# bastienjossen/DDL25Spring

Measured on AMD Instinct MI355X. Metric: FedAvg rounds/sec + local samples/sec, ResNet-18 CIFAR-10-shape, 8 clients, higher is better.
Workload: dtype fp32; 1 GPU; model=resnet18-cifar10, global_batch=800, parallelism=fedavg-8clients-dp1, clients=8, local_batch=100, local_epochs=1, samples_per_client=6250, client_slots_per_gpu=8, hip_graphs=True, fp32_conv_math=auto

## Files before the change

csrc/include/conv_f32_core.h:

```cpp
#pragma once
#include "ddl_common.h"

struct ConvF32Args {
  const float* x;
  const float* w;
  const float* dy;
  float* out;
  float* stats;
  const float* bias;
  const float* residual;
  const float* mask;
  const float* in_scale;
  const float* in_shift;
  const float* bn_x;
  const float* bn_mean;
  const float* bn_rstd;
  const float* mask_scale;
  const float* mask_shift;
  float* partial;
  long long partial_cap;
  long long x_gs, w_gs, dy_gs, out_gs, bias_gs, res_gs;
  int G, N, H, W, C, K, R, S, P, Q, stride, pad;
  int relu, accumulate, split_k, res_sub, in_relu;
  int slots;
  float gscale;
  const void* wsplit;
  long long ws_gs;
  const float* dyb_x;
  const float* dyb_coef;
  float* dyb_out;
  int* tickets;
  long long tickets_cap;
};

enum { F_FWD = 0, F_DGRAD = 1, F_WGRAD = 2 };

struct FDiv {
  uint32_t m;
  int s;
};
__host__ __device__ inline FDiv mk_fdiv(uint32_t d) {
  FDiv f;
  if (d <= 1) { f.m = 0; f.s = 0; return f; }
  int l = 0;
  while ((1u << l) < d) ++l;
  f.m = (uint32_t)((((1ull << 32) * ((1ull << l) - d)) / d) + 1);
  f.s = l;
  return f;
}
__device__ __forceinline__ int fdv(int x, FDiv f) {
  if (f.s == 0) return x;
  const uint32_t t = __umulhi((uint32_t)x, f.m);
  return (int)((t + (((uint32_t)x - t) >> 1)) >> (f.s - 1));
}

struct FGeo {
  int Pd, Qd, Kr, nph, phase, split, nsplit, g, p0, q0, tq;
  int pa, pb, Hs, Ws, r0, s0, Rn, Sn;
};

template <int MODE, int BP, int BQ>
__device__ __forceinline__ FGeo fgeo(const ConvF32Args& a, int bx, int by, int g, int gy) {
  FGeo o;
  o.nph = (MODE == F_DGRAD && a.stride == 2) ? 4 : 1;
  o.phase = by % o.nph;
  o.split = by / o.nph;
  o.nsplit = gy / o.nph;
  o.g = g;
  o.pa = o.pb = o.r0 = o.s0 = 0;
  o.Hs = a.H; o.Ws = a.W; o.Rn = a.R; o.Sn = a.S;
  if (MODE == F_FWD) {
    o.Pd = a.K; o.Qd = a.N * a.P * a.Q; o.Kr = a.R * a.S * a.C;
  } else if (MODE == F_DGRAD) {
    o.Pd = a.C;
    if (o.nph == 4) {
      o.pa = o.phase >> 1; o.pb = o.phase & 1;
      o.Hs = (a.H - o.pa + 1) >> 1; o.Ws = (a.W - o.pb + 1) >> 1;
      o.r0 = (o.pa + a.pad) & 1; o.s0 = (o.pb + a.pad) & 1;
      o.Rn = (a.R - o.r0 + 1) >> 1; o.Sn = (a.S - o.s0 + 1) >> 1;
    }
    o.Qd = a.N * o.Hs * o.Ws;
    o.Kr = o.Rn * o.Sn * a.K;
  } else {
    o.Pd = a.K; o.Qd = a.R * a.S * a.C; o.Kr = a.N * a.P * a.Q;
  }
  const int ntp = (o.Pd + BP - 1) / BP;
  o.p0 = (bx % ntp) * BP;
  o.tq = bx / ntp;
  o.q0 = o.tq * BQ;
  return o;
}

template <int BP, int BQ>
struct Lay16 {
  static constexpr int NPQ = BP / 32, NQ = BQ / 32, QL = 16;
  static __device__ __forceinline__ int poff(int i, int lane) { return i * 16 + 4 * (lane >> 4); }
  static __device__ __forceinline__ int qoff(int j, int lane) { return j * 16 + (lane & 15); }
};
template <int BP, int BQ>
struct Lay32 {
  static constexpr int NPQ = BP / 16, NQ = BQ / 64, QL = 32;
  static __device__ __forceinline__ int poff(int i, int lane) {
    return (i >> 2) * 32 + 8 * (i & 3) + 4 * (lane >> 5);
  }
  static __device__ __forceinline__ int qoff(int j, int lane) { return j * 32 + (lane & 31); }
};

template <int MODE, int BP, int BQ, class L>
__device__ __forceinline__ void fepi(const ConvF32Args& a, const FGeo& o, f4v (&acc)[L::NPQ][L::NQ], float* red) {
  constexpr int WP = BP / 2, WQ = BQ / 2, NP = L::NPQ, NQ = L::NQ, QL = L::QL;
  const int tid = threadIdx.x, lane = tid & 63, wid = tid >> 6, wp = wid >> 1, wq = wid & 1;
  const int g = o.g;
  if constexpr (MODE == F_WGRAD) {
    const int RSC = o.Qd;
    float* outg = a.out + (long long)g * a.out_gs;
#pragma unroll
    for (int i = 0; i < NP; ++i)
#pragma unroll
      for (int j = 0; j < NQ; ++j) {
        const int q = o.q0 + wq * WQ + L::qoff(j, lane);
        if (q >= RSC) continue;
#pragma unroll
        for (int v = 0; v < 4; ++v) {
          const int p = o.p0 + wp * WP + L::poff(i, lane) + v;
          if (p >= o.Pd) continue;
          float* d = outg + (long long)p * RSC + q;
          const float base = a.accumulate ? *d : 0.f;
          *d = base + a.gscale * acc[i][j][v];
        }
      }
    return;
  }
  const bool want_stats = a.stats != nullptr;
  const bool dg_stats = MODE == F_DGRAD && want_stats && a.bn_x;
  const int Pd = o.Pd;
  float* outg = a.out + (long long)g * a.out_gs;
  long long pix[NQ];
  int hq[NQ], wqq[NQ], nq_[NQ];
  bool qv[NQ];
  const FDiv dpq = mk_fdiv((uint32_t)(o.Hs * o.Ws)), dq = mk_fdiv((uint32_t)o.Ws);
#pragma unroll
  for (int j = 0; j < NQ; ++j) {
    const int q = o.q0 + wq * WQ + L::qoff(j, lane);
    qv[j] = q < o.Qd;
    pix[j] = q;
    hq[j] = wqq[j] = nq_[j] = 0;
    if (MODE == F_DGRAD) {
      const int nn = fdv(q, dpq);
      const int rem = q - nn * o.Hs * o.Ws;
      const int ii = fdv(rem, dq), jj = rem - ii * o.Ws;
      const int hh = o.nph == 4 ? 2 * ii + o.pa : ii;
      const int ww = o.nph == 4 ? 2 * jj + o.pb : jj;
      nq_[j] = nn; hq[j] = hh; wqq[j] = ww;
      pix[j] = ((long long)nn * a.H + hh) * a.W + ww;
    }
  }
#pragma unroll
  for (int i = 0; i < NP; ++i) {
    const int p = o.p0 + wp * WP + L::poff(i, lane);
    const bool pv = p < Pd;
    float bia[4], bm[4], br[4], ms[4], mh[4];
#pragma unroll
    for (int v = 0; v < 4; ++v) {
      bia[v] = (MODE == F_FWD && a.bias && pv) ? a.bias[(long long)g * a.bias_gs + p + v] : 0.f;
      bm[v] = (MODE == F_DGRAD && a.bn_x && pv) ? a.bn_mean[(long long)g * Pd + p + v] : 0.f;
      br[v] = (MODE == F_DGRAD && a.bn_x && pv) ? a.bn_rstd[(long long)g * Pd + p + v] : 0.f;
      ms[v] = (MODE == F_DGRAD && a.mask_scale && pv) ? a.mask_scale[(long long)g * Pd + p + v] : 0.f;
      mh[v] = (MODE == F_DGRAD && a.mask_scale && pv) ? a.mask_shift[(long long)g * Pd + p + v] : 0.f;
    }
    float s0[4] = {0.f, 0.f, 0.f, 0.f}, s1[4] = {0.f, 0.f, 0.f, 0.f};
    const float4 z4 = make_float4(0.f, 0.f, 0.f, 0.f);
    float4 rr[NQ], mm[NQ], xx[NQ];
    long long ee[NQ];
#pragma unroll
    for (int j = 0; j < NQ; ++j) ee[j] = (qv[j] && pv) ? pix[j] * Pd + p : 0;
    const long long gofs = (long long)g * a.out_gs;
    if (a.residual && (MODE == F_FWD || a.res_sub != 2)) {
#pragma unroll
      for (int j = 0; j < NQ; ++j) rr[j] = *(const float4*)(a.residual + gofs + ee[j]);
    } else if (MODE == F_DGRAD && a.residual) {
      const int Hc = (a.H + 1) >> 1, Wc = (a.W + 1) >> 1;
#pragma unroll
      for (int j = 0; j < NQ; ++j) {
        const bool on = qv[j] && pv && ((hq[j] | wqq[j]) & 1) == 0;
        const long long re = on ? (((long long)nq_[j] * Hc + (hq[j] >> 1)) * Wc + (wqq[j] >> 1)) * Pd + p : 0;
        rr[j] = *(const float4*)(a.residual + (long long)g * a.res_gs + re);
        if (!on) rr[j] = z4;
      }
    }
    if (MODE == F_DGRAD && a.mask) {
#pragma unroll
      for (int j = 0; j < NQ; ++j) mm[j] = *(const float4*)(a.mask + gofs + ee[j]);
    }
    if (MODE == F_DGRAD && a.bn_x) {
#pragma unroll
      for (int j = 0; j < NQ; ++j) xx[j] = *(const float4*)(a.bn_x + gofs + ee[j]);
    }
#pragma unroll
    for (int j = 0; j < NQ; ++j) {
      if (!qv[j] || !pv) continue;
      const long long e = ee[j];
      float v4[4] = {acc[i][j][0], acc[i][j][1], acc[i][j][2], acc[i][j][3]};
      if (MODE == F_FWD) {
#pragma unroll
        for (int v = 0; v < 4; ++v) v4[v] += bia[v];
        if (a.residual) {
          v4[0] += rr[j].x; v4[1] += rr[j].y; v4[2] += rr[j].z; v4[3] += rr[j].w;
        }
        if (a.relu) {
#pragma unroll
          for (int v = 0; v < 4; ++v) v4[v] = fmaxf(v4[v], 0.f);
        }
        if (want_stats) {
#pragma unroll
          for (int v = 0; v < 4; ++v) {
            s0[v] += v4[v];
            acc[i][j][v] = v4[v];
          }
        }
      } else {
        if (a.residual) {
          v4[0] += rr[j].x; v4[1] += rr[j].y; v4[2] += rr[j].z; v4[3] += rr[j].w;
        }
        if (a.mask) {
          const float4 m = mm[j];
          if (!(m.x > 0.f)) v4[0] = 0.f;
          if (!(m.y > 0.f)) v4[1] = 0.f;
          if (!(m.z > 0.f)) v4[2] = 0.f;
          if (!(m.w > 0.f)) v4[3] = 0.f;
        }
        if (a.bn_x) {
          const float xs[4] = {xx[j].x, xx[j].y, xx[j].z, xx[j].w};
          if (a.mask_scale) {
#pragma unroll
            for (int v = 0; v < 4; ++v)
              if (!(xs[v] * ms[v] + mh[v] > 0.f)) v4[v] = 0.f;
          }
          if (want_stats) {
#pragma unroll
            for (int v = 0; v < 4; ++v) {
              s0[v] += v4[v];
              s1[v] += v4[v] * ((xs[v] - bm[v]) * br[v]);
            }
          }
        }
      }
      *(float4*)(outg + e) = make_float4(v4[0], v4[1], v4[2], v4[3]);
    }
    if ((MODE == F_FWD && want_stats) || dg_stats) {
#pragma unroll
      for (int v = 0; v < 4; ++v) {
        float x0 = s0[v], x1 = s1[v];
#pragma unroll
        for (int o2 = 1; o2 < QL; o2 <<= 1) {
          x0 += __shfl_xor(x0, o2, 64);
          if (MODE == F_DGRAD) x1 += __shfl_xor(x1, o2, 64);
        }
        if ((lane & (QL - 1)) == 0) {
          const int pl = wp * WP + L::poff(i, lane) + v;
          red[(wq * BP + pl) * 2] = x0;
          if (MODE == F_DGRAD) red[(wq * BP + pl) * 2 + 1] = x1;
        }
      }
    }
  }
  if (!want_stats || (MODE == F_DGRAD && !a.bn_x)) return;
  if constexpr (MODE == F_FWD) {
    const int nq = min(BQ, o.Qd - o.q0);
    __syncthreads();
#pragma unroll
    for (int i = 0; i < NP; ++i) {
      const bool pv = o.p0 + wp * WP + L::poff(i, lane) < Pd;
      float mu[4], s1[4] = {0.f, 0.f, 0.f, 0.f};
#pragma unroll
      for (int v = 0; v < 4; ++v) {
        const int pl = wp * WP + L::poff(i, lane) + v;
        mu[v] = (red[pl * 2] + red[(BP + pl) * 2]) / (float)nq;
      }
#pragma unroll
      for (int j = 0; j < NQ; ++j) {
        if (!qv[j] || !pv) continue;
#pragma unroll
        for (int v = 0; v < 4; ++v) {
          const float d = acc[i][j][v] - mu[v];
          s1[v] += d * d;
        }
      }
#pragma unroll
      for (int v = 0; v < 4; ++v) {
        float x1 = s1[v];
#pragma unroll
        for (int o2 = 1; o2 < QL; o2 <<= 1) x1 += __shfl_xor(x1, o2, 64);
        if ((lane & (QL - 1)) == 0) red[(wq * BP + wp * WP + L::poff(i, lane) + v) * 2 + 1] = x1;
      }
    }
    __syncthreads();
    if (tid < BP && o.p0 + tid < Pd) {
      const int slot = o.phase * (a.slots / o.nph) + o.tq;
      float* st = a.stats + ((long long)g * a.slots + slot) * 2 * Pd + o.p0 + tid;
      st[0] = red[tid * 2] + red[(BP + tid) * 2];
      st[Pd] = red[tid * 2 + 1] + red[(BP + tid) * 2 + 1];
    }
    return;
  }
  __syncthreads();
  if (tid < BP && o.p0 + tid < Pd) {
    const float t0 = red[tid * 2] + red[(BP + tid) * 2];
    const float t1 = red[tid * 2 + 1] + red[(BP + tid) * 2 + 1];
    const int slot = o.phase * (a.slots / o.nph) + o.tq;
    float* st = a.stats + ((long long)g * a.slots + slot) * 2 * Pd + o.p0 + tid;
    st[0] = t0;
    st[Pd] = t1;
  }
}

template <int MODE, int BP>
__device__ __forceinline__ void fzero_slot(const ConvF32Args& a, const FGeo& o) {
  if (MODE == F_WGRAD || !a.stats || (MODE == F_DGRAD && !a.bn_x)) return;
  const int tid = threadIdx.x;
  if (tid < BP && o.p0 + tid < o.Pd) {
    const int slot = o.phase * (a.slots / o.nph) + o.tq;
    float* st = a.stats + ((long long)o.g * a.slots + slot) * 2 * o.Pd + o.p0 + tid;
    st[0] = 0.f;
    st[o.Pd] = 0.f;
  }
}

template <int MODE, int BP, int BQ>
__global__ __launch_bounds__(256) void convf32_splitk_epilogue(ConvF32Args a) {
  constexpr int WP = BP / 2, WQ = BQ / 2, TP = WP / 16, TQ = WQ / 16;
  __shared__ float red[2 * BP * 2];
  const int tid = threadIdx.x, lane = tid & 63, wid = tid >> 6, wp = wid >> 1, wq = wid & 1;
  const int nph = (MODE == F_DGRAD && a.stride == 2) ? 4 : 1;
  const FGeo o = fgeo<MODE, BP, BQ>(a, blockIdx.x, blockIdx.y, blockIdx.z, nph * a.split_k);
  if (o.q0 >= o.Qd || o.p0 >= o.Pd) {
    fzero_slot<MODE, BP>(a, o);
    return;
  }
  const long long qmax = (long long)a.slots / nph * BQ;
  const long long slice = (long long)a.G * nph * qmax * o.Pd;
  const float* base = a.partial + ((long long)o.g * nph + o.phase) * qmax * o.Pd;
  f4v acc[TP][TQ];
  bool ok[TP][TQ];
  const float* src[TP][TQ];
#pragma unroll
  for (int ti = 0; ti < TP; ++ti)
#pragma unroll
    for (int tj = 0; tj < TQ; ++tj) {
      const int q = o.q0 + wq * WQ + tj * 16 + (lane & 15);
      const int p = o.p0 + wp * WP + ti * 16 + 4 * (lane >> 4);
      ok[ti][tj] = q < o.Qd && p < o.Pd;
      src[ti][tj] = base + (ok[ti][tj] ? (long long)q * o.Pd + p : 0);
      acc[ti][tj] = (f4v){0.f, 0.f, 0.f, 0.f};
    }
  for (int k = 0; k < a.split_k; ++k) {
    f4v v[TP][TQ];
#pragma unroll
    for (int ti = 0; ti < TP; ++ti)
#pragma unroll
      for (int tj = 0; tj < TQ; ++tj)
        v[ti][tj] = ok[ti][tj] ? *(const f4v*)(src[ti][tj] + k * slice) : (f4v){0.f, 0.f, 0.f, 0.f};
#pragma unroll
    for (int ti = 0; ti < TP; ++ti)
#pragma unroll
      for (int tj = 0; tj < TQ; ++tj) acc[ti][tj] += v[ti][tj];
  }
  fepi<MODE, BP, BQ, Lay16<BP, BQ>>(a, o, acc, red);
}


__device__ __forceinline__ void split3(float4 v, s4v& h, s4v& m, s4v& l) {
  const float x[4] = {v.x, v.y, v.z, v.w};
#pragma unroll
  for (int i = 0; i < 4; ++i) {
    const uint32_t u = __float_as_uint(x[i]);
    const float r1 = x[i] - __uint_as_float(u & 0xFFFF0000u);
    const uint32_t um = __float_as_uint(r1);
    const float r2 = r1 - __uint_as_float(um & 0xFFFF0000u);
    h[i] = (short)(u >> 16);
    m[i] = (short)(um >> 16);
    l[i] = (short)(__float_as_uint(r2) >> 16);
  }
}
__device__ __forceinline__ void split1(float x, uint16_t& h, uint16_t& m, uint16_t& l) {
  const uint32_t u = __float_as_uint(x);
  const float r1 = x - __uint_as_float(u & 0xFFFF0000u);
  const uint32_t um = __float_as_uint(r1);
  const float r2 = r1 - __uint_as_float(um & 0xFFFF0000u);
  h = (uint16_t)(u >> 16);
  m = (uint16_t)(um >> 16);
  l = (uint16_t)(__float_as_uint(r2) >> 16);
}
__device__ __forceinline__ s8v cat44(s4v a, s4v b) {
  return __builtin_shufflevector(a, b, 0, 1, 2, 3, 4, 5, 6, 7);
}
```

csrc/kernels/conv_f32.hip:

```cpp
#include "conv_f32_core.h"
#include <cstdlib>

#ifndef F32_PREFETCH
#define F32_PREFETCH 2
#endif

constexpr int FBK = 16;

__device__ __forceinline__ int fswz(int row) { return (row >> 2) & 2; }
__device__ __forceinline__ int lds_off(int row, int ch) { return row * 16 + ((ch ^ fswz(row)) << 2); }

__device__ __forceinline__ int x6_off(int row, int ch, int half) {
  const int f = row & 2;
  const int g = (row ^ (row >> 2)) & 1;
  return row * 32 + 8 * (ch ^ f) + 4 * (half ^ g);
}

template <int MODE, int BP, int BQ, int X6>
__global__ __launch_bounds__(256, (X6 && BP * BQ <= 64 * 128) ? 3 : 2) void convf32_kernel(ConvF32Args a) {
  constexpr int WP = BP / 2, WQ = BQ / 2, TP = WP / 16, TQ = WQ / 16;
  constexpr int RW = X6 ? 32 : 16;
  constexpr int SP = BP * RW, SQ = BQ * RW;
  constexpr int UPK = BP / 64, UQK = BQ / 64;
  constexpr int KUP = BP / 64, KUQ = BQ / 64;
  __shared__ float4 smem4[(2 * (SP + SQ)) / 4];
  float* smem = (float*)smem4;
  __shared__ float xform[2 * 512];

  const int tid = threadIdx.x, lane = tid & 63, wid = tid >> 6, wp = wid >> 1, wq = wid & 1;
  const int gx = gridDim.x, gy = gridDim.y, gz = gridDim.z;
  const int lin = blockIdx.x + gx * (blockIdx.y + gy * blockIdx.z);
  const int u = xcd_remap(lin, gx * gy * gz);
  const int bx = u % gx, by = (u / gx) % gy, g = u / (gx * gy);
  const FGeo o = fgeo<MODE, BP, BQ>(a, bx, by, g, gy);
  const bool split_store = a.split_k > 1;
  if (o.q0 >= o.Qd || o.p0 >= o.Pd) {
    if (!split_store || (a.tickets && o.split == 0)) fzero_slot<MODE, BP>(a, o);
    return;
  }
  const int nk = (o.Kr + FBK - 1) / FBK;
  const int per = (nk + o.nsplit - 1) / o.nsplit;
  const int kt0 = o.split * per, kt1 = min(nk, kt0 + per);

  const int H = a.H, W = a.W, C = a.C, K = a.K, S = a.S, P = a.P, Q = a.Q, st = a.stride, pd = a.pad;
  const float* X = a.x + (long long)g * a.x_gs;
  const float* Wt = a.w + (long long)g * a.w_gs;
  const float* DY = a.dy + (long long)g * a.dy_gs;
  const bool xf = (MODE != F_DGRAD) && a.in_scale != nullptr;
  if (xf) {
    for (int i = tid; i < C; i += 256) {
      xform[i] = a.in_scale[(long long)g * C + i];
      xform[512 + i] = a.in_shift[(long long)g * C + i];
    }
  }
  const bool xrelu = a.in_relu != 0;

  int pk_row[UPK], pk_ch[UPK];
  int pm_rg = 0, pm_kp = 0;
  if constexpr (MODE == F_FWD) {
#pragma unroll
    for (int i = 0; i < UPK; ++i) {
      const int uu = tid + 256 * i;
      pk_row[i] = uu >> 2;
      pk_ch[i] = uu & 3;
    }
  } else {
    pm_kp = tid % (16 / KUP);
    pm_rg = tid / (16 / KUP);
  }
  int qk_row[UQK], qk_ch[UQK], qk_n[UQK], qk_hb[UQK], qk_wb[UQK];
  int qm_rg = 0, qm_kp = 0, qm_r = 0, qm_s = 0, qm_c = 0;
  bool qm_ok = false;
  float qm_sc[4] = {1.f, 1.f, 1.f, 1.f}, qm_sh[4] = {0.f, 0.f, 0.f, 0.f};
  if constexpr (MODE != F_WGRAD) {
    const FDiv dpq = mk_fdiv((uint32_t)(MODE == F_FWD ? P * Q : o.Hs * o.Ws));
    const FDiv dq = mk_fdiv((uint32_t)(MODE == F_FWD ? Q : o.Ws));
    const int PQ = MODE == F_FWD ? P * Q : o.Hs * o.Ws, QQ = MODE == F_FWD ? Q : o.Ws;
#pragma unroll
    for (int i = 0; i < UQK; ++i) {
      const int uu = tid + 256 * i;
      qk_row[i] = uu >> 2;
      qk_ch[i] = uu & 3;
      const int q = o.q0 + qk_row[i];
      if (q < o.Qd) {
        const int n = fdv(q, dpq), rem = q - n * PQ;
        const int y = fdv(rem, dq), xq = rem - y * QQ;
        qk_n[i] = n;
        if (MODE == F_FWD) {
          qk_hb[i] = y * st - pd;
          qk_wb[i] = xq * st - pd;
        } else {
          qk_hb[i] = (o.nph == 4 ? 2 * y + o.pa : y) + pd;
          qk_wb[i] = (o.nph == 4 ? 2 * xq + o.pb : xq) + pd;
        }
      } else {
        qk_n[i] = -1;
        qk_hb[i] = qk_wb[i] = 0;
      }
    }
  } else {
    qm_kp = tid % (16 / KUQ);
    qm_rg = tid / (16 / KUQ);
    const int q = o.q0 + 4 * qm_rg;
    qm_ok = q < o.Qd;
    if (qm_ok) {
      const int tap = q / C;
      qm_c = q - tap * C;
      qm_r = tap / S;
      qm_s = tap - qm_r * S;
    }
  }
  if (xf) __syncthreads();
  if constexpr (MODE == F_WGRAD) {
    if (xf && qm_ok) {
#pragma unroll
      for (int v = 0; v < 4; ++v) { qm_sc[v] = xform[qm_c + v]; qm_sh[v] = xform[512 + qm_c + v]; }
    }
  }
  const FDiv dpix = mk_fdiv((uint32_t)(P * Q)), dpq1 = mk_fdiv((uint32_t)Q);

  constexpr unsigned OOB = 0xFFFFFFF0u;
  const __amdgpu_buffer_rsrc_t rX = __builtin_amdgcn_make_buffer_rsrc(
      (void*)X, 0, (int)((long long)a.N * H * W * C * 4), 0x00020000);
  const __amdgpu_buffer_rsrc_t rW = __builtin_amdgcn_make_buffer_rsrc(
      (void*)Wt, 0, (int)((long long)K * a.R * S * C * 4), 0x00020000);
  const __amdgpu_buffer_rsrc_t rD = __builtin_amdgcn_make_buffer_rsrc(
      (void*)DY, 0, (int)((long long)a.N * P * Q * K * 4), 0x00020000);
  auto bload = [&](const __amdgpu_buffer_rsrc_t& rs, unsigned off) -> float4 {
    const auto v = __builtin_amdgcn_raw_buffer_load_b128(rs, off, 0, 0);
    return __builtin_bit_cast(float4, v);
  };
  constexpr int PF = F32_PREFETCH;
  float4 rpA[2], rqA[2], rpB[2], rqB[2], rpC[2], rqC[2];
  bool qvA[2] = {false, false}, qvB[2] = {false, false}, qvC[2] = {false, false};
  auto load_step = [&](int kt, float4 (&rp)[2], float4 (&rq)[2], bool (&qv)[2]) {
    const int kk0 = kt * FBK;
    if constexpr (MODE == F_FWD) {
#pragma unroll
      for (int i = 0; i < UPK; ++i) {
        const int p = o.p0 + pk_row[i];
        rp[i] = bload(rW, p < o.Pd ? (unsigned)(p * o.Kr + kk0 + 4 * pk_ch[i]) * 4u : OOB);
      }
    } else if constexpr (MODE == F_DGRAD) {
      const int tap = kk0 / K, k0 = kk0 - tap * K;
      const int ir = tap / o.Sn, is = tap - ir * o.Sn;
      const int r = o.r0 + (st == 2 ? 2 : 1) * ir, s = o.s0 + (st == 2 ? 2 : 1) * is;
      const int c = o.p0 + 4 * pm_rg;
#pragma unroll
      for (int j = 0; j < KUP; ++j) {
        const int k = k0 + pm_kp * KUP + j;
        rp[j] = bload(rW, c < C ? (unsigned)(((k * a.R + r) * S + s) * C + c) * 4u : OOB);
      }
    } else {
      const int kch = o.p0 + 4 * pm_rg;
#pragma unroll
      for (int j = 0; j < KUP; ++j) {
        const int pix = kk0 + pm_kp * KUP + j;
        rp[j] = bload(rD, (pix < o.Kr && kch < K) ? (unsigned)(pix * K + kch) * 4u : OOB);
      }
    }
    if constexpr (MODE == F_FWD) {
      const int tap = kk0 / C, c0 = kk0 - tap * C;
      const int r = tap / S, s = tap - r * S;
#pragma unroll
      for (int i = 0; i < UQK; ++i) {
        const int h = qk_hb[i] + r, w = qk_wb[i] + s;
        const bool ok = qk_n[i] >= 0 && (unsigned)h < (unsigned)H && (unsigned)w < (unsigned)W;
        qv[i] = ok;
        rq[i] = bload(rX, ok ? (unsigned)(((qk_n[i] * H + h) * W + w) * C + c0 + 4 * qk_ch[i]) * 4u : OOB);
      }
    } else if constexpr (MODE == F_DGRAD) {
      const int tap = kk0 / K, k0 = kk0 - tap * K;
      const int ir = tap / o.Sn, is = tap - ir * o.Sn;
      const int r = o.r0 + (st == 2 ? 2 : 1) * ir, s = o.s0 + (st == 2 ? 2 : 1) * is;
#pragma unroll
      for (int i = 0; i < UQK; ++i) {
        int ho = qk_hb[i] - r, wo = qk_wb[i] - s;
        bool hit = true;
        if (st == 2) {
          ho >>= 1;
          wo >>= 1;
        } else if (st > 2) {
          hit = ho >= 0 && wo >= 0 && ho % st == 0 && wo % st == 0;
          ho /= st;
          wo /= st;
        }
        const bool ok = hit && qk_n[i] >= 0 && (unsigned)ho < (unsigned)P && (unsigned)wo < (unsigned)Q;
        rq[i] = bload(rD, ok ? (unsigned)(((qk_n[i] * P + ho) * Q + wo) * K + k0 + 4 * qk_ch[i]) * 4u : OOB);
      }
    } else {
#pragma unroll
      for (int j = 0; j < KUQ; ++j) {
        const int pix = kk0 + qm_kp * KUQ + j;
        const int n = fdv(pix, dpix), rem = pix - n * P * Q;
        const int ho = fdv(rem, dpq1), wo = rem - ho * Q;
        const int h = ho * st - pd + qm_r, w = wo * st - pd + qm_s;
        const bool ok = qm_ok && pix < o.Kr && (unsigned)h < (unsigned)H && (unsigned)w < (unsigned)W;
        qv[j] = ok;
        rq[j] = bload(rX, ok ? (unsigned)(((n * H + h) * W + w) * C + qm_c) * 4u : OOB);
      }
    }
  };
  auto xform4 = [&](float4 v, const float* sc, const float* sh) {
    v.x = v.x * sc[0] + sh[0];
    v.y = v.y * sc[1] + sh[1];
    v.z = v.z * sc[2] + sh[2];
    v.w = v.w * sc[3] + sh[3];
    if (xrelu) { v.x = fmaxf(v.x, 0.f); v.y = fmaxf(v.y, 0.f); v.z = fmaxf(v.z, 0.f); v.w = fmaxf(v.w, 0.f); }
    return v;
  };
  auto store_mn = [&](float* img, int rg, int kp, int KU, const float4* v) {
#pragma unroll
    for (int j4 = 0; j4 < 4; ++j4) {
      const int row = 4 * rg + j4;
      const int kk = kp * KU;
      float* d = img + row * 16 + (((kk >> 2) ^ fswz(row)) << 2) + (kk & 3);
      const float e0 = j4 == 0 ? v[0].x : j4 == 1 ? v[0].y : j4 == 2 ? v[0].z : v[0].w;
      if (KU == 2) {
        const float e1 = j4 == 0 ? v[1].x : j4 == 1 ? v[1].y : j4 == 2 ? v[1].z : v[1].w;
        *(float2*)d = make_float2(e0, e1);
      } else {
        *d = e0;
      }
    }
  };
  auto store_k6 = [&](float* img, int row, int ch, float4 v) {
    s4v h, m, l;
    split3(v, h, m, l);
    *(s8v*)(img + x6_off(row, ch, 0)) = cat44(h, m);
    *(s8v*)(img + x6_off(row, ch, 1)) = cat44(l, h);
  };
  auto store_mn6 = [&](float* img, int rg, int kp, int KU, const float4* v) {
#pragma unroll
    for (int j4 = 0; j4 < 4; ++j4) {
      const int row = 4 * rg + j4;
      const int kk = kp * KU, ch = kk >> 2, pos = kk & 3;
      uint16_t* h0 = (uint16_t*)(img + x6_off(row, ch, 0)) + pos;
      uint16_t* h1 = (uint16_t*)(img + x6_off(row, ch, 1)) + pos;
      const float e0 = j4 == 0 ? v[0].x : j4 == 1 ? v[0].y : j4 == 2 ? v[0].z : v[0].w;
      uint16_t ah, am, al;
      split1(e0, ah, am, al);
      if (KU == 2) {
        const float e1 = j4 == 0 ? v[1].x : j4 == 1 ? v[1].y : j4 == 2 ? v[1].z : v[1].w;
        uint16_t bh, bm, bl;
        split1(e1, bh, bm, bl);
        *(uint32_t*)h0 = (uint32_t)ah | ((uint32_t)bh << 16);
        *(uint32_t*)(h0 + 4) = (uint32_t)am | ((uint32_t)bm << 16);
        *(uint32_t*)h1 = (uint32_t)al | ((uint32_t)bl << 16);
        *(uint32_t*)(h1 + 4) = (uint32_t)ah | ((uint32_t)bh << 16);
      } else {
        h0[0] = ah;
        h0[4] = am;
        h1[0] = al;
        h1[4] = ah;
      }
    }
  };
  auto store_step = [&](int buf, int kt, float4 (&rp)[2], float4 (&rq)[2], const bool (&qv)[2]) {
    float* Ps = smem + buf * (SP + SQ);
    float* Qs = Ps + SP;
    if constexpr (MODE == F_FWD) {
#pragma unroll
      for (int i = 0; i < UPK; ++i) {
        if constexpr (X6) store_k6(Ps, pk_row[i], pk_ch[i], rp[i]);
        else *(float4*)(Ps + lds_off(pk_row[i], pk_ch[i])) = rp[i];
      }
    } else {
      if constexpr (X6) store_mn6(Ps, pm_rg, pm_kp, KUP, rp);
      else store_mn(Ps, pm_rg, pm_kp, KUP, rp);
    }
    if constexpr (MODE == F_FWD) {
      if (xf) {
        const int kk0 = kt * FBK, c0 = kk0 - (kk0 / C) * C;
#pragma unroll
        for (int i = 0; i < UQK; ++i) {
          const int c = c0 + 4 * qk_ch[i];
          if (qv[i]) rq[i] = xform4(rq[i], xform + c, xform + 512 + c);
        }
      }
    } else if constexpr (MODE == F_WGRAD) {
      if (xf) {
#pragma unroll
        for (int j = 0; j < KUQ; ++j)
          if (qv[j]) rq[j] = xform4(rq[j], qm_sc, qm_sh);
      }
    }
    if constexpr (MODE != F_WGRAD) {
#pragma unroll
      for (int i = 0; i < UQK; ++i) {
        if constexpr (X6) store_k6(Qs, qk_row[i], qk_ch[i], rq[i]);
        else *(float4*)(Qs + lds_off(qk_row[i], qk_ch[i])) = rq[i];
      }
    } else {
      if constexpr (X6) store_mn6(Qs, qm_rg, qm_kp, KUQ, rq);
      else store_mn(Qs, qm_rg, qm_kp, KUQ, rq);
    }
  };

  f4v acc[TP][TQ];
#pragma unroll
  for (int i = 0; i < TP; ++i)
#pragma unroll
    for (int j = 0; j < TQ; ++j) acc[i][j] = (f4v){0.f, 0.f, 0.f, 0.f};

  auto step = [&](int kt, float4 (&cp)[2], float4 (&cq)[2], bool (&cv)[2], float4 (&np)[2],
                  float4 (&nq)[2], bool (&nv)[2]) {
    const int cur = (kt - kt0) & 1;
    if (kt + PF < kt1) load_step(kt + PF, np, nq, nv);
    const float* Ps = smem + cur * (SP + SQ);
    const float* Qs = Ps + SP;
    if constexpr (X6) {
      s8v a0[TP], a1[TP], b0[TQ], b1[TQ];
#pragma unroll
      for (int ti = 0; ti < TP; ++ti) {
        const int R = wp * WP + ti * 16 + (lane & 15);
        a0[ti] = *(const s8v*)(Ps + x6_off(R, lane >> 4, 0));
        a1[ti] = *(const s8v*)(Ps + x6_off(R, lane >> 4, 1));
      }
#pragma unroll
      for (int tj = 0; tj < TQ; ++tj) {
        const int R = wq * WQ + tj * 16 + (lane & 15);
        b0[tj] = *(const s8v*)(Qs + x6_off(R, lane >> 4, 0));
        b1[tj] = *(const s8v*)(Qs + x6_off(R, lane >> 4, 1));
      }
#pragma unroll
      for (int ti = 0; ti < TP; ++ti)
#pragma unroll
        for (int tj = 0; tj < TQ; ++tj) {
          f4v c = __builtin_amdgcn_mfma_f32_16x16x32_bf16(a1[ti], b0[tj], (f4v){0.f, 0.f, 0.f, 0.f}, 0, 0, 0);
          c = __builtin_amdgcn_mfma_f32_16x16x32_bf16(a0[ti], b1[tj], c, 0, 0, 0);
          c = __builtin_amdgcn_mfma_f32_16x16x32_bf16(a0[ti], b0[tj], c, 0, 0, 0);
#pragma unroll
          for (int v = 0; v < 4; ++v) acc[ti][tj][v] = acc[ti][tj][v] + c[v];
        }
    } else {
      float4 af[TP], bfr[TQ];
#pragma unroll
      for (int ti = 0; ti < TP; ++ti)
        af[ti] = *(const float4*)(Ps + lds_off(wp * WP + ti * 16 + (lane & 15), lane >> 4));
#pragma unroll
      for (int tj = 0; tj < TQ; ++tj)
        bfr[tj] = *(const float4*)(Qs + lds_off(wq * WQ + tj * 16 + (lane & 15), lane >> 4));
#pragma unroll
      for (int s4 = 0; s4 < 4; ++s4)
#pragma unroll
        for (int ti = 0; ti < TP; ++ti)
#pragma unroll
          for (int tj = 0; tj < TQ; ++tj) {
            const float av = s4 == 0 ? af[ti].x : s4 == 1 ? af[ti].y : s4 == 2 ? af[ti].z : af[ti].w;
            const float bv = s4 == 0 ? bfr[tj].x : s4 == 1 ? bfr[tj].y : s4 == 2 ? bfr[tj].z : bfr[tj].w;
            acc[ti][tj] = __builtin_amdgcn_mfma_f32_16x16x4f32(av, bv, acc[ti][tj], 0, 0, 0);
          }
    }
    if (kt + 1 < kt1) store_step(cur ^ 1, kt + 1, cp, cq, cv);
    __syncthreads();
  };
  if (kt0 < kt1) {
    load_step(kt0, rpA, rqA, qvA);
    if (kt0 + 1 < kt1) load_step(kt0 + 1, rpB, rqB, qvB);
    if constexpr (PF == 3) {
      if (kt0 + 2 < kt1) load_step(kt0 + 2, rpC, rqC, qvC);
    }
    store_step(0, kt0, rpA, rqA, qvA);
    __syncthreads();
    if constexpr (PF == 3) {
      for (int kt = kt0; kt < kt1; kt += 3) {
        step(kt, rpB, rqB, qvB, rpA, rqA, qvA);
        if (kt + 1 < kt1) step(kt + 1, rpC, rqC, qvC, rpB, rqB, qvB);
        if (kt + 2 < kt1) step(kt + 2, rpA, rqA, qvA, rpC, rqC, qvC);
      }
    } else {
      for (int kt = kt0; kt < kt1; kt += 2) {
        step(kt, rpB, rqB, qvB, rpA, rqA, qvA);
        if (kt + 1 < kt1) step(kt + 1, rpA, rqA, qvA, rpB, rqB, qvB);
      }
    }
  }

  if (split_store) {
#pragma unroll
    for (int ti = 0; ti < TP; ++ti)
#pragma unroll
      for (int tj = 0; tj < TQ; ++tj) {
        const int q = o.q0 + wq * WQ + tj * 16 + (lane & 15);
        const int p = o.p0 + wp * WP + ti * 16 + 4 * (lane >> 4);
        if (q >= o.Qd || p >= o.Pd) continue;
        if constexpr (MODE == F_WGRAD) {
          float* d = a.partial + ((long long)o.split * a.G + g) * o.Pd * o.Qd;
#pragma unroll
          for (int v = 0; v < 4; ++v)
            if (p + v < o.Pd) d[(long long)(p + v) * o.Qd + q] = acc[ti][tj][v];
        } else {
          const long long qmax = (long long)a.slots / o.nph * BQ;
          float* d = a.partial + (((long long)o.split * a.G + g) * o.nph + o.phase) * qmax * o.Pd;
          *(float4*)(d + (long long)q * o.Pd + p) = make_float4(acc[ti][tj][0], acc[ti][tj][1],
                                                                acc[ti][tj][2], acc[ti][tj][3]);
        }
      }
    if (a.tickets) {
      __threadfence();
      __syncthreads();
      int* const last = (int*)smem;
      int* const ticket = a.tickets + ((long long)g * o.nph + o.phase) * gx + bx;
      if (tid == 0) *last = atomicAdd(ticket, 1) == o.nsplit - 1;
      __syncthreads();
      if (!*last) return;
      __threadfence();
      if constexpr (MODE != F_WGRAD) {
        const long long qmax = (long long)a.slots / o.nph * BQ;
        const long long slice = (long long)a.G * o.nph * qmax * o.Pd;
        const float* base = a.partial + ((long long)g * o.nph + o.phase) * qmax * o.Pd;
#pragma unroll
        for (int ti = 0; ti < TP; ++ti)
#pragma unroll
          for (int tj = 0; tj < TQ; ++tj) {
            const int q = o.q0 + wq * WQ + tj * 16 + (lane & 15);
            const int p = o.p0 + wp * WP + ti * 16 + 4 * (lane >> 4);
            f4v sm = (f4v){0.f, 0.f, 0.f, 0.f};
            if (q < o.Qd && p < o.Pd) {
              const float* src = base + (long long)q * o.Pd + p;
              for (int k = 0; k < o.nsplit; ++k) {
                const float4 v = *(const float4*)(src + k * slice);
                sm[0] += v.x; sm[1] += v.y; sm[2] += v.z; sm[3] += v.w;
              }
            }
            acc[ti][tj] = sm;
          }
        __syncthreads();
        if (tid == 0) *ticket = 0;
        fepi<MODE, BP, BQ, Lay16<BP, BQ>>(a, o, acc, smem);
        return;
      } else {
        const long long per = (long long)o.Pd * o.Qd;
        const float* src = a.partial + (long long)g * per;
        float* dst = a.out + (long long)g * a.out_gs;
        for (int e = tid; e < BP * (BQ / 4); e += 256) {
          const int p = o.p0 + e / (BQ / 4), q = o.q0 + 4 * (e % (BQ / 4));
          if (p >= o.Pd || q >= o.Qd) continue;
          const long long off = (long long)p * o.Qd + q;
          float4 sum = make_float4(0.f, 0.f, 0.f, 0.f);
          for (int k = 0; k < o.nsplit; ++k) {
            const float4 v = *(const float4*)(src + (long long)k * a.G * per + off);
            sum.x += v.x; sum.y += v.y; sum.z += v.z; sum.w += v.w;
          }
          float4 b = a.accumulate ? *(const float4*)(dst + off) : make_float4(0.f, 0.f, 0.f, 0.f);
          b.x += a.gscale * sum.x; b.y += a.gscale * sum.y; b.z += a.gscale * sum.z; b.w += a.gscale * sum.w;
          *(float4*)(dst + off) = b;
        }
        if (tid == 0) *ticket = 0;
      }
    }
    return;
  }
  fepi<MODE, BP, BQ, Lay16<BP, BQ>>(a, o, acc, smem);
}

template <int V>
__global__ __launch_bounds__(256) void convf32_wgrad_reduce(const float* __restrict__ part, float* out,
                                                            long long out_gs, int G, long long nv,
                                                            int splits, int accumulate, float gscale) {
  typedef float vec __attribute__((ext_vector_type(V)));
  const long long per = nv * V;
  GSTRIDE_LOOP(t, (long long)G * nv) {
    const long long g = t / nv, i = (t - g * nv) * V;
    vec s = (vec)(0.f);
    const float* src = part + g * per + i;
    const long long sstride = (long long)G * per;
    int k = 0;
    for (; k + 8 <= splits; k += 8) {
      vec v[8];
#pragma unroll
      for (int j = 0; j < 8; ++j) v[j] = *(const vec*)(src + (long long)(k + j) * sstride);
#pragma unroll
      for (int j = 0; j < 8; ++j) s += v[j];
    }
    for (; k < splits; ++k) s += *(const vec*)(src + (long long)k * sstride);
    float* d = out + g * out_gs + i;
    vec b = accumulate ? *(const vec*)d : (vec)(0.f);
    b += gscale * s;
    *(vec*)d = b;
  }
}

static void launch_wgrad_reduce(const float* part, float* out, long long out_gs, int G, long long n, int splits,
                                int accumulate, float gscale, hipStream_t s) {
  static const long long v4_min = [] {
    const char* e = getenv("DDL_WGRAD_REDUCE_V4_MIN");
    return e ? atoll(e) : 512LL * 256;
  }();
  if ((long long)G * (n / 4) >= v4_min)
    hipLaunchKernelGGL(convf32_wgrad_reduce<4>, dim3(grid_for((long long)G * (n / 4), 256)), dim3(256), 0, s, part,
                       out, out_gs, G, n / 4, splits, accumulate, gscale);
  else
    hipLaunchKernelGGL(convf32_wgrad_reduce<1>, dim3(grid_for((long long)G * n, 256)), dim3(256), 0, s, part, out,
                       out_gs, G, n, splits, accumulate, gscale);
}

DDL_API int ddl_convf32_wgrad_reduce(const float* part, float* out, long long out_gs, int G, long long n, int splits,
                                     int accumulate, float gscale, hipStream_t s) {
  if (n % 4) return (int)hipErrorInvalidValue;
  launch_wgrad_reduce(part, out, out_gs, G, n, splits, accumulate, gscale, s);
  return (int)hipGetLastError();
}

static void fdims(const ConvF32Args& a, int mode, long long& Pd, long long& Qd, long long& Qmax, long long& Kr,
                  int& nph) {
  nph = (mode == F_DGRAD && a.stride == 2) ? 4 : 1;
  if (mode == F_FWD) { Pd = a.K; Qd = Qmax = (long long)a.N * a.P * a.Q; Kr = (long long)a.R * a.S * a.C; }
  else if (mode == F_DGRAD) {
    Pd = a.C;
    const int Hs = nph == 4 ? (a.H + 1) >> 1 : a.H, Ws = nph == 4 ? (a.W + 1) >> 1 : a.W;
    Qd = Qmax = (long long)a.N * Hs * Ws;
    Kr = (long long)a.R * a.S * a.K;
  } else { Pd = a.K; Qd = Qmax = (long long)a.R * a.S * a.C; Kr = (long long)a.N * a.P * a.Q; }
}

DDL_API long long ddl_convf32_slots(const ConvF32Args* ap, int mode, int cfg) {
  long long Pd, Qd, Qmax, Kr;
  int nph;
  fdims(*ap, mode, Pd, Qd, Qmax, Kr, nph);
  const int bq = ((cfg >> 8) & 0xff) * 16;
  if (bq <= 0) return -1;
  return nph * ((Qmax + bq - 1) / bq);
}

DDL_API long long ddl_convf32_workspace(const ConvF32Args* ap, int mode, int cfg) {
  if (ap->split_k <= 1) return 0;
  long long Pd, Qd, Qmax, Kr;
  int nph;
  fdims(*ap, mode, Pd, Qd, Qmax, Kr, nph);
  const int bq = ((cfg >> 8) & 0xff) * 16;
  if (mode == F_WGRAD) return (long long)ap->split_k * ap->G * Pd * Qd;
  const long long qm = (Qmax + bq - 1) / bq * bq;
  return (long long)ap->split_k * ap->G * nph * qm * Pd;
}

template <int MODE, int BP, int BQ, int X6>
static int launch_tile(ConvF32Args a, hipStream_t s) {
  long long Pd, Qd, Qmax, Kr;
  int nph;
  fdims(a, MODE, Pd, Qd, Qmax, Kr, nph);
  const long long ntp = (Pd + BP - 1) / BP, ntq = (Qmax + BQ - 1) / BQ;
  a.slots = (int)(nph * ntq);
  const int split = a.split_k < 1 ? 1 : a.split_k;
  a.split_k = split;
  if (split > 1) {
    const long long need = MODE == F_WGRAD ? (long long)split * a.G * Pd * Qd
                                           : (long long)split * a.G * nph * ntq * BQ * Pd;
    if (!a.partial || need > a.partial_cap) return (int)hipErrorInvalidValue;
  }
  const dim3 grid((unsigned)(ntp * ntq), (unsigned)(nph * split), (unsigned)a.G);
  if (split == 1 || (long long)a.G * nph * ntp * ntq > a.tickets_cap) a.tickets = nullptr;
  hipLaunchKernelGGL((convf32_kernel<MODE, BP, BQ, X6>), grid, dim3(256), 0, s, a);
  hipError_t e = hipGetLastError();
  if (e != hipSuccess || split == 1 || a.tickets) return (int)e;
  if (MODE == F_WGRAD) {
    launch_wgrad_reduce((const float*)a.partial, a.out, a.out_gs, a.G, Pd * Qd, split, a.accumulate, a.gscale, s);
  } else {
    hipLaunchKernelGGL((convf32_splitk_epilogue<MODE, BP, BQ>), dim3((unsigned)(ntp * ntq), nph, a.G),
                       dim3(256), 0, s, a);
  }
  return (int)hipGetLastError();
}

template <int MODE, int X6>
static int launch_math(const ConvF32Args& a, int bp, int bq, hipStream_t s) {
  if (bp == 64 && bq == 64) return launch_tile<MODE, 64, 64, X6>(a, s);
  if (bp == 64 && bq == 128) return launch_tile<MODE, 64, 128, X6>(a, s);
  if (bp == 128 && bq == 64) return launch_tile<MODE, 128, 64, X6>(a, s);
  if (bp == 128 && bq == 128) return launch_tile<MODE, 128, 128, X6>(a, s);
  return (int)hipErrorInvalidValue;
}

template <int MODE>
static int launch_mode(const ConvF32Args& a, int cfg, hipStream_t s) {
  const int bp = (cfg & 0xff) * 16, bq = ((cfg >> 8) & 0xff) * 16;
  return (cfg >> 16) & 1 ? launch_math<MODE, 1>(a, bp, bq, s) : launch_math<MODE, 0>(a, bp, bq, s);
}

DDL_API int ddl_convf32(const ConvF32Args* ap, int mode, int cfg, hipStream_t s) {
  const ConvF32Args& a = *ap;
  if (a.G < 1 || a.N < 1 || a.C < 1 || a.K < 1 || a.stride < 1) return (int)hipErrorInvalidValue;
  if (a.C > 512 && a.in_scale) return (int)hipErrorInvalidValue;
  const long long lim = (1LL << 31) - 64;
  if ((long long)a.N * a.H * a.W * a.C * 4 > lim || (long long)a.K * a.R * a.S * a.C * 4 > lim ||
      (long long)a.N * a.P * a.Q * a.K * 4 > lim)
    return (int)hipErrorInvalidValue;
  if (mode == F_FWD) {
    if (a.C % 16 || a.K % 4) return (int)hipErrorInvalidValue;
    return launch_mode<F_FWD>(a, cfg, s);
  }
  if (mode == F_DGRAD) {
    if (a.K % 16 || a.C % 4) return (int)hipErrorInvalidValue;
    return launch_mode<F_DGRAD>(a, cfg, s);
  }
  if (mode == F_WGRAD) {
    if (a.C % 4 || a.K % 4) return (int)hipErrorInvalidValue;
    if (!a.accumulate && a.gscale != 1.f) return (int)hipErrorInvalidValue;
    return launch_mode<F_WGRAD>(a, cfg, s);
  }
  return (int)hipErrorInvalidValue;
}

DDL_API int ddl_convf32_args_size() { return (int)sizeof(ConvF32Args); }
```

Baseline: 42500 samples/s.

## Replace per-step index divisions with incremental address walkers in fp32 conv

Precomputes base buffer offsets per thread and advances tap, channel and pixel positions incrementally instead of recomputing divisions and multiplications on every k-step in forward, dgrad and wgrad loaders. The bf16x3 split stores now pack halves with v_perm into 128-bit stores, and the input transform becomes branchless selects. This targets integer ALU and address overhead in the load path. The incremental walkers assume k-steps advance sequentially by FBK and carry logic stays correct for every shape; dropping the batch-index bound checks relies on the NEVER sentinel.

Result: no change. 42920 samples/s (median of 6 runs) (+1.0%).

```diff
diff --git a/csrc/include/conv_f32_core.h b/csrc/include/conv_f32_core.h
--- a/csrc/include/conv_f32_core.h
+++ b/csrc/include/conv_f32_core.h
@@ -391,6 +391,25 @@
   m = (uint16_t)(um >> 16);
   l = (uint16_t)(__float_as_uint(r2) >> 16);
 }
+__device__ __forceinline__ void split1w(float x, uint32_t& h, uint32_t& m, uint32_t& l) {
+  h = __float_as_uint(x);
+  const float r1 = x - __uint_as_float(h & 0xFFFF0000u);
+  m = __float_as_uint(r1);
+  l = __float_as_uint(r1 - __uint_as_float(m & 0xFFFF0000u));
+}
+__device__ __forceinline__ uint32_t pack_hi16(uint32_t lo, uint32_t hi) {
+  return __builtin_amdgcn_perm(hi, lo, 0x07060302u);
+}
+__device__ __forceinline__ void split3_halves(float4 v, uint4& hm, uint4& lh) {
+  uint32_t h[4], m[4], l[4];
+  split1w(v.x, h[0], m[0], l[0]);
+  split1w(v.y, h[1], m[1], l[1]);
+  split1w(v.z, h[2], m[2], l[2]);
+  split1w(v.w, h[3], m[3], l[3]);
+  const uint32_t h01 = pack_hi16(h[0], h[1]), h23 = pack_hi16(h[2], h[3]);
+  hm = make_uint4(h01, h23, pack_hi16(m[0], m[1]), pack_hi16(m[2], m[3]));
+  lh = make_uint4(pack_hi16(l[0], l[1]), pack_hi16(l[2], l[3]), h01, h23);
+}
 __device__ __forceinline__ s8v cat44(s4v a, s4v b) {
   return __builtin_shufflevector(a, b, 0, 1, 2, 3, 4, 5, 6, 7);
 }
diff --git a/csrc/include/conv_f32_walk.h b/csrc/include/conv_f32_walk.h
--- /dev/null
+++ b/csrc/include/conv_f32_walk.h
@@ -0,0 +1,78 @@
+#pragma once
+
+#if defined(__HIPCC__)
+#define F32W_FN __host__ __device__ __forceinline__
+#else
+#define F32W_FN inline
+#endif
+
+struct PixStride {
+  int st;
+  int w_adv, h_adv;
+  int w_span, h_span;
+  unsigned off_adv;
+  unsigned off_one;
+  unsigned off_wcarry;
+  unsigned off_hcarry;
+};
+
+struct PixPos {
+  int h, w;
+  unsigned off;
+};
+
+F32W_FN PixStride mk_pixstride(int H, int W, int C, int P, int Q, int st) {
+  const int PQ = P * Q, a = 16 / PQ, b = 16 - a * PQ, c = b / Q, d = b - c * Q;
+  PixStride s;
+  s.st = st;
+  s.w_adv = d * st;
+  s.h_adv = c * st;
+  s.w_span = Q * st;
+  s.h_span = P * st;
+  s.off_adv = (unsigned)((a * H + c * st) * W + d * st) * (unsigned)C * 4u;
+  s.off_one = (unsigned)(st * C) * 4u;
+  s.off_wcarry = (unsigned)((st * W - Q * st) * C) * 4u;
+  s.off_hcarry = (unsigned)((H - P * st) * W * C) * 4u;
+  return s;
+}
+
+F32W_FN void pix_advance(PixPos& p, int w_add, int h_add, unsigned off_add, int wmax, int hmax, const PixStride& s) {
+  p.w += w_add;
+  p.h += h_add;
+  p.off += off_add;
+  const bool cw = p.w >= wmax;
+  p.w = cw ? p.w - s.w_span : p.w;
+  p.h = cw ? p.h + s.st : p.h;
+  p.off = cw ? p.off + s.off_wcarry : p.off;
+  const bool ch = p.h >= hmax;
+  p.h = ch ? p.h - s.h_span : p.h;
+  p.off = ch ? p.off + s.off_hcarry : p.off;
+}
+F32W_FN void pix_step(PixPos& p, int wmax, int hmax, const PixStride& s) {
+  pix_advance(p, s.w_adv, s.h_adv, s.off_adv, wmax, hmax, s);
+}
+F32W_FN void pix_one(PixPos& p, int wmax, int hmax, const PixStride& s) {
+  pix_advance(p, s.st, 0, s.off_one, wmax, hmax, s);
+}
+
+struct TapWalk {
+  int tr, ts, c0;
+};
+F32W_FN TapWalk mk_tapwalk(int kk0, int NS, int NC) {
+  TapWalk t;
+  const int tap = kk0 / NC;
+  t.c0 = kk0 - tap * NC;
+  t.tr = tap / NS;
+  t.ts = tap - t.tr * NS;
+  return t;
+}
+F32W_FN void tap_step(TapWalk& t, int NS, int NC) {
+  t.c0 += 16;
+  if (t.c0 >= NC) {
+    t.c0 = 0;
+    if (++t.ts >= NS) {
+      t.ts = 0;
+      ++t.tr;
+    }
+  }
+}
diff --git a/csrc/kernels/conv_f32.hip b/csrc/kernels/conv_f32.hip
--- a/csrc/kernels/conv_f32.hip
+++ b/csrc/kernels/conv_f32.hip
@@ -1,4 +1,5 @@
 #include "conv_f32_core.h"
+#include "conv_f32_walk.h"
 #include <cstdlib>
 
 #ifndef F32_PREFETCH
@@ -55,23 +56,43 @@
   }
   const bool xrelu = a.in_relu != 0;
 
+  constexpr unsigned FAR = 0x80000000u;
+  constexpr int NEVER = -(1 << 30);
   int pk_row[UPK], pk_ch[UPK];
+  unsigned pk_off[UPK];
   int pm_rg = 0, pm_kp = 0;
+  unsigned pm_off = 0;
+  unsigned pm_adv = 0;
   if constexpr (MODE == F_FWD) {
 #pragma unroll
     for (int i = 0; i < UPK; ++i) {
       const int uu = tid + 256 * i;
       pk_row[i] = uu >> 2;
       pk_ch[i] = uu & 3;
+      const int p = o.p0 + pk_row[i];
+      pk_off[i] = p < o.Pd ? (unsigned)(p * o.Kr + 4 * pk_ch[i]) * 4u : FAR;
     }
   } else {
     pm_kp = tid % (16 / KUP);
     pm_rg = tid / (16 / KUP);
-  }
-  int qk_row[UQK], qk_ch[UQK], qk_n[UQK], qk_hb[UQK], qk_wb[UQK];
-  int qm_rg = 0, qm_kp = 0, qm_r = 0, qm_s = 0, qm_c = 0;
+    const int pc = o.p0 + 4 * pm_rg;
+    if constexpr (MODE == F_DGRAD) {
+      pm_off = pc < C ? (unsigned)(pm_kp * KUP * a.R * S * C + pc) * 4u : FAR;
+    } else {
+      pm_off = pc < K ? (unsigned)((kt0 * FBK + pm_kp * KUP) * K + pc) * 4u : FAR;
+      pm_adv = pc < K ? (unsigned)(FBK * K) * 4u : 0u;
+    }
+  }
+  int qk_row[UQK], qk_ch[UQK], qk_hb[UQK], qk_wb[UQK];
+  unsigned qk_off[UQK];
+  int qm_rg = 0, qm_kp = 0, qm_c = 0;
   bool qm_ok = false;
   float qm_sc[4] = {1.f, 1.f, 1.f, 1.f}, qm_sh[4] = {0.f, 0.f, 0.f, 0.f};
+  TapWalk tw = {0, 0, 0};
+  int st_c0 = 0;
+  PixStride pxs = {};
+  PixPos qpos = {0, 0, 0};
+  int q_hmax = 0, q_wmax = 0, q_lpix = 0;
   if constexpr (MODE != F_WGRAD) {
     const FDiv dpq = mk_fdiv((uint32_t)(MODE == F_FWD ? P * Q : o.Hs * o.Ws));
     const FDiv dq = mk_fdiv((uint32_t)(MODE == F_FWD ? Q : o.Ws));
@@ -85,30 +106,45 @@
       if (q < o.Qd) {
         const int n = fdv(q, dpq), rem = q - n * PQ;
         const int y = fdv(rem, dq), xq = rem - y * QQ;
-        qk_n[i] = n;
         if (MODE == F_FWD) {
           qk_hb[i] = y * st - pd;
           qk_wb[i] = xq * st - pd;
+          qk_off[i] = (unsigned)(((n * H + qk_hb[i]) * W + qk_wb[i]) * C + 4 * qk_ch[i]) * 4u;
         } else {
           qk_hb[i] = (o.nph == 4 ? 2 * y + o.pa : y) + pd;
           qk_wb[i] = (o.nph == 4 ? 2 * xq + o.pb : xq) + pd;
+          qk_off[i] = (unsigned)(n * P * Q * K + 4 * qk_ch[i]) * 4u;
         }
       } else {
-        qk_n[i] = -1;
-        qk_hb[i] = qk_wb[i] = 0;
-      }
-    }
+        qk_hb[i] = qk_wb[i] = NEVER;
+        qk_off[i] = 0;
+      }
+    }
+    tw = mk_tapwalk(kt0 * FBK, MODE == F_FWD ? S : o.Sn, MODE == F_FWD ? C : K);
+    st_c0 = tw.c0;
   } else {
     qm_kp = tid % (16 / KUQ);
     qm_rg = tid / (16 / KUQ);
     const int q = o.q0 + 4 * qm_rg;
     qm_ok = q < o.Qd;
+    int qm_r = 0, qm_s = 0;
     if (qm_ok) {
       const int tap = q / C;
       qm_c = q - tap * C;
       qm_r = tap / S;
       qm_s = tap - qm_r * S;
     }
+    const FDiv dpix = mk_fdiv((uint32_t)(P * Q)), dpq1 = mk_fdiv((uint32_t)Q);
+    const int pix = kt0 * FBK + qm_kp * KUQ;
+    const int n = fdv(pix, dpix), rem = pix - n * P * Q;
+    const int ho = fdv(rem, dpq1), wo = rem - ho * Q;
+    pxs = mk_pixstride(H, W, C, P, Q, st);
+    qpos.h = ho * st - pd + qm_r;
+    qpos.w = wo * st - pd + qm_s;
+    qpos.off = (unsigned)(((n * H + qpos.h) * W + qpos.w) * C + qm_c) * 4u;
+    q_hmax = P * st - pd + qm_r;
+    q_wmax = Q * st - pd + qm_s;
+    q_lpix = qm_ok ? qm_kp * KUQ : -NEVER;
   }
   if (xf) __syncthreads();
   if constexpr (MODE == F_WGRAD) {
@@ -117,7 +153,6 @@
       for (int v = 0; v < 4; ++v) { qm_sc[v] = xform[qm_c + v]; qm_sh[v] = xform[512 + qm_c + v]; }
     }
   }
-  const FDiv dpix = mk_fdiv((uint32_t)(P * Q)), dpq1 = mk_fdiv((uint32_t)Q);
 
   constexpr unsigned OOB = 0xFFFFFFF0u;
   const __amdgpu_buffer_rsrc_t rX = __builtin_amdgcn_make_buffer_rsrc(
@@ -136,43 +171,26 @@
   auto load_step = [&](int kt, float4 (&rp)[2], float4 (&rq)[2], bool (&qv)[2]) {
     const int kk0 = kt * FBK;
     if constexpr (MODE == F_FWD) {
-#pragma unroll
-      for (int i = 0; i < UPK; ++i) {
-        const int p = o.p0 + pk_row[i];
-        rp[i] = bload(rW, p < o.Pd ? (unsigned)(p * o.Kr + kk0 + 4 * pk_ch[i]) * 4u : OOB);
-      }
-    } else if constexpr (MODE == F_DGRAD) {
-      const int tap = kk0 / K, k0 = kk0 - tap * K;
-      const int ir = tap / o.Sn, is = tap - ir * o.Sn;
-      const int r = o.r0 + (st == 2 ? 2 : 1) * ir, s = o.s0 + (st == 2 ? 2 : 1) * is;
-      const int c = o.p0 + 4 * pm_rg;
-#pragma unroll
-      for (int j = 0; j < KUP; ++j) {
-        const int k = k0 + pm_kp * KUP + j;
-        rp[j] = bload(rW, c < C ? (unsigned)(((k * a.R + r) * S + s) * C + c) * 4u : OOB);
-      }
-    } else {
-      const int kch = o.p0 + 4 * pm_rg;
-#pragma unroll
-      for (int j = 0; j < KUP; ++j) {
-        const int pix = kk0 + pm_kp * KUP + j;
-        rp[j] = bload(rD, (pix < o.Kr && kch < K) ? (unsigned)(pix * K + kch) * 4u : OOB);
-      }
-    }
-    if constexpr (MODE == F_FWD) {
-      const int tap = kk0 / C, c0 = kk0 - tap * C;
-      const int r = tap / S, s = tap - r * S;
+      const unsigned wstep = (unsigned)kk0 * 4u;
+#pragma unroll
+      for (int i = 0; i < UPK; ++i) rp[i] = bload(rW, pk_off[i] + wstep);
+      const int r = tw.tr, s = tw.ts;
+      const unsigned xtap = (unsigned)((r * W + s) * C + tw.c0) * 4u;
 #pragma unroll
       for (int i = 0; i < UQK; ++i) {
         const int h = qk_hb[i] + r, w = qk_wb[i] + s;
-        const bool ok = qk_n[i] >= 0 && (unsigned)h < (unsigned)H && (unsigned)w < (unsigned)W;
+        const bool ok = ((unsigned)h < (unsigned)H) & ((unsigned)w < (unsigned)W);
         qv[i] = ok;
-        rq[i] = bload(rX, ok ? (unsigned)(((qk_n[i] * H + h) * W + w) * C + c0 + 4 * qk_ch[i]) * 4u : OOB);
-      }
+        rq[i] = bload(rX, ok ? qk_off[i] + xtap : OOB);
+      }
+      tap_step(tw, S, C);
     } else if constexpr (MODE == F_DGRAD) {
-      const int tap = kk0 / K, k0 = kk0 - tap * K;
-      const int ir = tap / o.Sn, is = tap - ir * o.Sn;
+      const int ir = tw.tr, is = tw.ts, k0 = tw.c0;
       const int r = o.r0 + (st == 2 ? 2 : 1) * ir, s = o.s0 + (st == 2 ? 2 : 1) * is;
+      const unsigned wtap = (unsigned)(((k0 * a.R + r) * S + s) * C) * 4u;
+      const unsigned wk = (unsigned)(a.R * S * C) * 4u;
+#pragma unroll
+      for (int j = 0; j < KUP; ++j) rp[j] = bload(rW, pm_off + wtap + (unsigned)j * wk);
 #pragma unroll
       for (int i = 0; i < UQK; ++i) {
         int ho = qk_hb[i] - r, wo = qk_wb[i] - s;
@@ -185,28 +203,37 @@
           ho /= st;
           wo /= st;
         }
-        const bool ok = hit && qk_n[i] >= 0 && (unsigned)ho < (unsigned)P && (unsigned)wo < (unsigned)Q;
-        rq[i] = bload(rD, ok ? (unsigned)(((qk_n[i] * P + ho) * Q + wo) * K + k0 + 4 * qk_ch[i]) * 4u : OOB);
-      }
+        const bool ok = hit && (unsigned)ho < (unsigned)P && (unsigned)wo < (unsigned)Q;
+        rq[i] = bload(rD, ok ? qk_off[i] + (unsigned)((ho * Q + wo) * K + k0) * 4u : OOB);
+      }
+      tap_step(tw, o.Sn, K);
     } else {
 #pragma unroll
+      for (int j = 0; j < KUP; ++j) rp[j] = bload(rD, pm_off + (unsigned)(j * K) * 4u);
+      pm_off += pm_adv;
+      const int left = o.Kr - kk0;
+      PixPos px = qpos;
+#pragma unroll
       for (int j = 0; j < KUQ; ++j) {
-        const int pix = kk0 + qm_kp * KUQ + j;
-        const int n = fdv(pix, dpix), rem = pix - n * P * Q;
-        const int ho = fdv(rem, dpq1), wo = rem - ho * Q;
-        const int h = ho * st - pd + qm_r, w = wo * st - pd + qm_s;
-        const bool ok = qm_ok && pix < o.Kr && (unsigned)h < (unsigned)H && (unsigned)w < (unsigned)W;
+        const bool ok = (q_lpix + j < left) & ((unsigned)px.h < (unsigned)H) & ((unsigned)px.w < (unsigned)W);
         qv[j] = ok;
-        rq[j] = bload(rX, ok ? (unsigned)(((n * H + h) * W + w) * C + qm_c) * 4u : OOB);
-      }
-    }
-  };
-  auto xform4 = [&](float4 v, const float* sc, const float* sh) {
-    v.x = v.x * sc[0] + sh[0];
-    v.y = v.y * sc[1] + sh[1];
-    v.z = v.z * sc[2] + sh[2];
-    v.w = v.w * sc[3] + sh[3];
-    if (xrelu) { v.x = fmaxf(v.x, 0.f); v.y = fmaxf(v.y, 0.f); v.z = fmaxf(v.z, 0.f); v.w = fmaxf(v.w, 0.f); }
+        rq[j] = bload(rX, ok ? px.off : OOB);
+        if (j + 1 < KUQ) pix_one(px, q_wmax, q_hmax, pxs);
+      }
+      pix_step(qpos, q_wmax, q_hmax, pxs);
+    }
+  };
+  auto xform4 = [&](float4 v, bool on, const float* sc, const float* sh) {
+    float4 t;
+    t.x = v.x * sc[0] + sh[0];
+    t.y = v.y * sc[1] + sh[1];
+    t.z = v.z * sc[2] + sh[2];
+    t.w = v.w * sc[3] + sh[3];
+    if (xrelu) { t.x = fmaxf(t.x, 0.f); t.y = fmaxf(t.y, 0.f); t.z = fmaxf(t.z, 0.f); t.w = fmaxf(t.w, 0.f); }
+    v.x = on ? t.x : v.x;
+    v.y = on ? t.y : v.y;
+    v.z = on ? t.z : v.z;
+    v.w = on ? t.w : v.w;
     return v;
   };
   auto store_mn = [&](float* img, int rg, int kp, int KU, const float4* v) {
@@ -225,10 +252,10 @@
     }
   };
   auto store_k6 = [&](float* img, int row, int ch, float4 v) {
-    s4v h, m, l;
-    split3(v, h, m, l);
-    *(s8v*)(img + x6_off(row, ch, 0)) = cat44(h, m);
-    *(s8v*)(img + x6_off(row, ch, 1)) = cat44(l, h);
+    uint4 hm, lh;
+    split3_halves(v, hm, lh);
+    *(uint4*)(img + x6_off(row, ch, 0)) = hm;
+    *(uint4*)(img + x6_off(row, ch, 1)) = lh;
   };
   auto store_mn6 = [&](float* img, int rg, int kp, int KU, const float4* v) {
 #pragma unroll
@@ -238,17 +265,19 @@
       uint16_t* h0 = (uint16_t*)(img + x6_off(row, ch, 0)) + pos;
       uint16_t* h1 = (uint16_t*)(img + x6_off(row, ch, 1)) + pos;
       const float e0 = j4 == 0 ? v[0].x : j4 == 1 ? v[0].y : j4 == 2 ? v[0].z : v[0].w;
-      uint16_t ah, am, al;
-      split1(e0, ah, am, al);
       if (KU == 2) {
         const float e1 = j4 == 0 ? v[1].x : j4 == 1 ? v[1].y : j4 == 2 ? v[1].z : v[1].w;
-        uint16_t bh, bm, bl;
-        split1(e1, bh, bm, bl);
-        *(uint32_t*)h0 = (uint32_t)ah | ((uint32_t)bh << 16);
-        *(uint32_t*)(h0 + 4) = (uint32_t)am | ((uint32_t)bm << 16);
-        *(uint32_t*)h1 = (uint32_t)al | ((uint32_t)bl << 16);
-        *(uint32_t*)(h1 + 4) = (uint32_t)ah | ((uint32_t)bh << 16);
+        uint32_t ah, am, al, bh, bm, bl;
+        split1w(e0, ah, am, al);
+        split1w(e1, bh, bm, bl);
+        const uint32_t hh = pack_hi16(ah, bh);
+        *(uint32_t*)h0 = hh;
+        *(uint32_t*)(h0 + 4) = pack_hi16(am, bm);
+        *(uint32_t*)h1 = pack_hi16(al, bl);
+        *(uint32_t*)(h1 + 4) = hh;
       } else {
+        uint16_t ah, am, al;
+        split1(e0, ah, am, al);
         h0[0] = ah;
         h0[4] = am;
         h1[0] = al;
@@ -271,18 +300,18 @@
     }
     if constexpr (MODE == F_FWD) {
       if (xf) {
-        const int kk0 = kt * FBK, c0 = kk0 - (kk0 / C) * C;
 #pragma unroll
         for (int i = 0; i < UQK; ++i) {
-          const int c = c0 + 4 * qk_ch[i];
-          if (qv[i]) rq[i] = xform4(rq[i], xform + c, xform + 512 + c);
+          const int c = st_c0 + 4 * qk_ch[i];
+          rq[i] = xform4(rq[i], qv[i], xform + c, xform + 512 + c);
         }
+        st_c0 += FBK;
+        if (st_c0 >= C) st_c0 = 0;
       }
     } else if constexpr (MODE == F_WGRAD) {
       if (xf) {
 #pragma unroll
-        for (int j = 0; j < KUQ; ++j)
-          if (qv[j]) rq[j] = xform4(rq[j], qm_sc, qm_sh);
+        for (int j = 0; j < KUQ; ++j) rq[j] = xform4(rq[j], qv[j], qm_sc, qm_sh);
       }
     }
     if constexpr (MODE != F_WGRAD) {
```
